# codeslake/RefVSR

Measured on AMD Instinct MI355X. Metric: 4x SR frames/sec (270p->1080p, RefVSR_small_L1), higher is better.
Workload: dtype f16; 1 GPU; config_RefVSR_small_L1 4x SR, 270x480 -> 1080x1920, frame_num=5, steady-state sliding window, n=1 (BASELINE configs[1]); synthetic clip seed 0, seeded random weights 1234; frames_per_rank=20, parallelism=frame-shard x1 (reset-aligned, no collective), window_cache=True, frame_ids=True, pipelined_calls=True, frames_per_call=4, headline_mode=frame groups, pipe_layout=pfm, full=False

## Files before the change

include/refvsr_hip.h:

```cpp
#ifndef REFVSR_HIP_H
#define REFVSR_HIP_H

#include <stddef.h>
#include <stdint.h>

#ifdef __cplusplus
extern "C" {
#endif

#define REFVSR_ABI_VERSION 15

int refvsr_abi_version(void);
int refvsr_max_maps(void);
const char* refvsr_last_error(void);
int refvsr_init(void);

int refvsr_num_cus(void);
int refvsr_stream_create_cu_range(int first_cu, int n_cus, void** stream);
int refvsr_stream_set_cu_budget(void* stream, int n_cus);
int refvsr_stream_destroy(void* stream);

enum { REFVSR_OUT_NHWC16 = 0, REFVSR_OUT_NHWC16_SHUFFLE2 = 1, REFVSR_OUT_PLANAR32 = 2 };

typedef struct RefvsrConv {
// ... 108 lines not shown
int refvsr_conf_alpha_f16w(const float* conf_a, const float* conf_b, int h, int w, int up, const float* w0, const float* b0,
                           float slope0, const void* blob, int cout, float slope1, void* alpha, float* conf_max, void* stream);
int refvsr_conf_alpha_batch_f16w(const float* const* conf_a, const float* const* conf_b, int batch, int h, int w, int up, const float* w0,
                                 const float* b0, float slope0, const void* blob, int cout, float slope1, void* const* alpha,
                                 float* const* conf_max, void* stream);
int refvsr_set_probe(void* buf, int iter);

int refvsr_conv_direct_f32(const float* src, int cin, int h, int w,
                           const float* wgt, const float* bias, int cout, int ksize, int stride, int pad,
                           float act_slope, void* out, int out_nhwc16, int out_c, void* stream);
int refvsr_conv1x1_f32(const float* src, int cin, int h, int w, const float* wgt, const float* bias, float act_slope,
                       float* out, void* stream);

int refvsr_pack_nhwc16(const float* src, int c, int h, int w, void* dst, int cs, void* stream);
int refvsr_pack_nhwc32(const float* src, int c, int h, int w, float* dst, int cs, void* stream);
int refvsr_unpack_nhwc16(const void* src, int h, int w, int cs, int c, float* dst, void* stream);

enum { REFVSR_RS_BICUBIC = 0, REFVSR_RS_BILINEAR = 1, REFVSR_RS_BILINEAR_AC = 2, REFVSR_RS_NEAREST = 3 };
int refvsr_resize(const float* src, int c, int h, int w, void* dst, int oh, int ow, int mode,
                  float src_scale_y, float src_scale_x, const float* mean, const float* std,
                  const float* chan_mul, int clamp01, int out_nhwc16, int out_c, void* stream);
int refvsr_avgpool2(const float* src, int c, int h, int w, float* dst, void* stream);
int refvsr_maxpool2(const float* src, int c, int h, int w, float* dst, void* stream);
int refvsr_buffers_equal(const void* const* a, const void* const* b, int n_pairs, size_t n_bytes,
                         int32_t* flags, void* stream);
int refvsr_bytes_equal(const void* const* a, const void* const* b, int n_pairs, size_t n_bytes,
                       int32_t* flags, void* stream);
int refvsr_max2(const float* a, const float* b, float* out, size_t n, void* stream);

#define REFVSR_INGEST_MAX_FRAMES 16
enum { REFVSR_INGEST_PLANAR = 0, REFVSR_INGEST_HWC = 1 };
int refvsr_ingest_u8(const void* const* src, float* const* dst, int nframes, int h, int w, int layout, void* stream);
int refvsr_ingest_table(float* out);
int refvsr_ingest_max_frames(void);

#define REFVSR_SCORE_MAX_FRAMES 16
size_t refvsr_score_workspace_bytes(int nframes, int h, int w);
int refvsr_score_max_frames(void);
int refvsr_score_frames(const void* const* out, int out_fmt, const void* const* gt, int gt_fmt, int gt_layout, int nframes, int h, int w,
                        int win, void* workspace, size_t workspace_bytes, double* scores, void* stream);

#define REFVSR_SCORE_MAX_RECTS 8
size_t refvsr_score_regions_workspace_bytes(int nframes, int h, int w, int nrects);
int refvsr_score_max_rects(void);
int refvsr_score_regions(const void* const* out, int out_fmt, const void* const* gt, int gt_fmt, int gt_layout, int nframes, int h, int w,
                         const int* rects, int nrects, void* workspace, size_t workspace_bytes, double* sums, void* stream);

int refvsr_warp_nhwc16(const void* x, int hin, int win, int cs, const float* flow, int hf, int wf,
                       void* out, void* stream);
int refvsr_warp_nhwc16_up2(const void* x, int hin, int win, int cs, const float* flow_lr, int hl, int wl,
                           void* out, void* stream);
int refvsr_warp_planar(const float* x, int c, int hin, int win, const float* flow, int hf, int wf,
                       float* out, void* stream);
int refvsr_warp_nhwc16_batch(const void* const* x, int batch, int hin, int win, int cs, const float* const* flow, int hf, int wf,
                             void* const* out, void* stream);
int refvsr_warp_nhwc16_up2_batch(const void* const* x, int batch, int hin, int win, int cs, const float* const* flow_lr, int hl, int wl,
                                 void* const* out, void* stream);
int refvsr_warp_planar_batch(const float* const* x, int batch, int c, int hin, int win, const float* const* flow, int hf, int wf,
                             float* const* out, void* stream);
int refvsr_spynet_level_input(const float* ref, const float* supp, const float* flow_prev, int h, int w,
                              void* out8, float* flow_up, void* stream);
int refvsr_spynet_level_input_batch(const float* const* ref, const float* const* supp, int batch, const float* flow_prev,
                                    int h, int w, void* out8, float* flow_up, void* stream);

#define REFVSR_MATCH_KP 152
#define REFVSR_MATCH_ROWCHUNK 256
#define REFVSR_MATCH_COLBLOCK 512
int refvsr_match_patches(const float* feat, int h, int w, void* rows, float* inv_norm, void* rows_lo, void* stream);
int refvsr_match_top2(const void* ref_rows, int n_ref, const void* lr_rows, int n_lr, int row_splits,
                      int32_t* cand_idx, float* cand_val, void* stream);
int refvsr_match_refine(const float* lr_feat, int h, int w, const float* ref_feat, int hr, int wr,
                        const float* inv_lr, const float* inv_ref, const int32_t* cand_idx, const float* cand_val,
                        int ncand, float margin, int32_t* flagged, float* conf, int32_t* idx, void* stream);
int refvsr_match_exact(const float* lr_feat, int h, int w, const float* ref_feat, int hr, int wr, const void* lr_rows,
                       const void* lr_rows_lo, const void* ref_rows, const void* ref_rows_lo, const float* inv_lr,
                       const float* inv_ref, const int32_t* flagged, void* keys, float* conf, int32_t* idx, void* stream);
int refvsr_match_naive(const float* lr_feat, int h, int w, const float* ref_feat, int hr, int wr,
                       float* conf, int32_t* idx, void* stream);

int refvsr_block_gather_nhwc16(const void* value, int hv, int wv, int cs, const int32_t* idx, int gh, int gw,
                               int s, void* out, void* stream);
int refvsr_block_gather_rgb(const float* value, int hv, int wv, const int32_t* idx, int gh, int gw, int s,
                            void* out8, float* out_planar, void* stream);
int refvsr_aligned_sample(const void* x, int h, int w, int ks, int cs, const float* affine, void* out,
                          void* stream);

int refvsr_dcn_sample(const void* x, int h, int w, int c, const float* offset_mask, int deform_groups, void* cols,
                      void* stream);
int refvsr_tsa_weight(const void* const* aligned, const void* const* emb, const void* emb_ref, int t, int c, int npix,
                      void* out, void* stream);
int refvsr_pool3s2_nhwc16(const void* x, int h, int w, int c, void* out, int out_c, int c_off, int is_max, void* stream);
// ... 8 lines not shown
```

refvsr_amd/csrc/match.hip:

```cpp
#include <stdlib.h>

#include "match_common.h"

#define LO_SCALE 2048.0f
#define LO_UNSCALE (1.0f / 2048.0f)

__global__ __launch_bounds__(128) void match_patches_kernel(const float* __restrict__ feat, int h, int w,
                                                            f16* __restrict__ rows, float* __restrict__ inv_norm,
                                                            f16* __restrict__ rows_lo) {
    __shared__ float s_inv[128];
    const int tid = threadIdx.x, p0 = blockIdx.x * 128, n = h * w;
    const size_t plane = (size_t)h * w;
    {
        const int p = min(p0 + tid, n - 1);
        const int y = p / w, x = p - y * w;
        int yy[3], xx[3];
#pragma unroll
        for (int k = 0; k < 3; ++k) { yy[k] = rv_reflect(y + k - 1, h) * w; xx[k] = rv_reflect(x + k - 1, w); }
        float ss = 0.0f;
        for (int c = 0; c < 16; ++c) {
            const float* f = feat + c * plane;
#pragma unroll
            for (int ky = 0; ky < 3; ++ky)
#pragma unroll
// ... 11 lines not shown
        const int y = p / w, x = p - y * w;
        const float inv = s_inv[pl];
        f16x8 o, lo;
#pragma unroll
        for (int k = 0; k < 8; ++k) {
            const int e = g * 8 + k;
            float v = 0.0f;
            if (e < 144) {
                const int c = e / 9, t = e - c * 9;
                const int ky = t / 3, kx = t - ky * 3;
                v = feat[c * plane + (size_t)rv_reflect(y + ky - 1, h) * w + rv_reflect(x + kx - 1, w)];
            }
            float vn = v * inv;
            asm volatile("" : "+v"(vn));
            o[k] = (f16)vn;
            lo[k] = (f16)((vn - (float)o[k]) * LO_SCALE);
        }
        const size_t off = (size_t)p0 * KP + (size_t)i * 8;
        *reinterpret_cast<f16x8*>(rows + off) = o;
        if (rows_lo) *reinterpret_cast<f16x8*>(rows_lo + off) = lo;
    }
}

extern "C" int refvsr_match_patches(const float* feat, int h, int w, void* rows, float* inv_norm, void* rows_lo,
                                    void* stream) {
    RV_CHECK(feat && rows && inv_norm && h >= 2 && w >= 2, "match_patches: bad args");
    hipLaunchKernelGGL(match_patches_kernel, dim3(rv_cdiv(h * w, 128)), dim3(128), 0, (hipStream_t)stream,
                       feat, h, w, (f16*)rows, inv_norm, (f16*)rows_lo);
    RV_LAUNCH_CHECK();
    return 0;
}

template <int UNROLL = 1>
__device__ __forceinline__ float patch_dot(const float* __restrict__ lf, int h, int w, const int* ly, const int* lx,
                                           const float* __restrict__ rf, int hr, int wr, int ry, int rx) {
    int yy[3], xx[3];
#pragma unroll
    for (int k = 0; k < 3; ++k) { yy[k] = rv_reflect(ry + k - 1, hr); xx[k] = rv_reflect(rx + k - 1, wr); }
    const size_t lp = (size_t)h * w, rp = (size_t)hr * wr;
    float d = 0.0f;
#pragma unroll 1
    for (int c0 = 0; c0 < 16; c0 += UNROLL) {
        float a[UNROLL][9], b[UNROLL][9];
#pragma unroll
        for (int u = 0; u < UNROLL; ++u)
#pragma unroll
            for (int t = 0; t < 9; ++t) {
                a[u][t] = lf[(c0 + u) * lp + (size_t)ly[t / 3] * w + lx[t % 3]];
                b[u][t] = rf[(c0 + u) * rp + (size_t)yy[t / 3] * wr + xx[t % 3]];
            }
#pragma unroll
// ... 265 lines not shown
```

refvsr_amd/engine.py:

```python
import collections
import itertools
import os

import torch

from . import ops
from .config import resolve_weight_precision
from .knobs import env_flag
from .packing import pack_conv
from .weights import VGG_MEAN, VGG_STD, round16

_uid = itertools.count()


def _timed_event(stream):
    e = torch.cuda.Event(enable_timing=True)
    e.record(stream)
    return e


def _flow_pairs(fr, restart):
    t = len(fr)
    ctr = t // 2
    need = [(fr[i], fr[i + 1]) for i in range(ctr, t - 1)] + [(fr[ctr + 1], fr[ctr])]
# ... 153 lines not shown
        self.nb = config.num_blocks
        self.ks = config.matching_ksize
        self.hd = bool(config.flag_HD_in)
        self.vgg7 = self.hd or config.scale != 4
        self.cache = bool(getattr(config, 'cache_windows', True))
        self.match_row_splits = 1
        self.match_margin = float(getattr(config, 'match_exact_margin', ops.MATCH_EXACT_MARGIN))
        self.chain_calls = bool(getattr(config, 'chain_calls', not env_flag('REFVSR_NO_CHAIN_CALLS')))
        self.fuse_resblocks = (bool(getattr(config, 'fuse_resblocks', True)) and ops.resblock_fits(self.C)
                               and not env_flag('REFVSR_NO_FUSE'))
        self.rb24 = not env_flag('REFVSR_NO_RB24')
        self.rb48 = (bool(getattr(config, 'fuse_resblocks', True)) and not env_flag('REFVSR_NO_FUSE')
                     and not env_flag('REFVSR_NO_RB48'))
        self.rb48_max_pixels = int(os.environ.get('REFVSR_RB48_MAX_PIXELS', str(540 * 960)))
        self.rb48_multimap = not env_flag('REFVSR_NO_RB48_MULTIMAP')
        self.spynet_mt1_pixels = int(os.environ.get('REFVSR_SPYNET_MT1_PIXELS', str(72 * 120)))
        self.bw_head_blocks = min(self.nb, max(-1, int(getattr(config, 'bw_head_blocks', None) if getattr(config, 'bw_head_blocks', None) is not None
                                                         else os.environ.get('REFVSR_BW_HEAD_BLOCKS', '12'))))
        self.warp_up2 = not env_flag('REFVSR_NO_WARP_UP2')
        self.fuse_head = not env_flag('REFVSR_NO_FUSE_HEAD')
        self.fuse_tail = self.fuse_head and (env_flag('REFVSR_FUSE_TAIL') or bool(getattr(config, 'fuse_tail', False)))
        self.fuse_conf = not env_flag('REFVSR_NO_FUSE_CONF')
        self.map1x1 = not env_flag('REFVSR_NO_MAP1X1')
        self.spynet_batch = not env_flag('REFVSR_NO_SPYNET_BATCH')
        self.overlap = bool(getattr(config, 'overlap_streams', True)) and not env_flag('REFVSR_NO_OVERLAP')
        self._side = None
        self.pipelined = bool(getattr(config, 'pipelined', False))
        self._zero_maps = {}
        self.result_dtype = str(getattr(config, 'result_dtype', None) or 'float32').replace('torch.', '')
        ops.result_format(self.result_dtype)
        self._pipe = None
        self._layout_default = None
        self.pipe_depth = max(1, int(getattr(config, 'pipe_depth', None) or os.environ.get('REFVSR_PIPE_DEPTH') or 3))
        self._inflight = collections.deque()
        self.stream_events = None
        self.kernel_events = None
        self.chain_events = None
        self.reset_state()

    def reset_state(self):
        self.fw_feat = None
        self.fw_flow = None
        self.fw_feat_up = None
        self.fw_conf = None
        self.frame_itr_num = 0
        self.max_frame_itr_num = self.cfg.reset_branch
# ... 256 lines not shown

    def res_list(self, x, name, n):
        pairs = [(self.cw('%s.RBs.%d.conv1' % (name, i)), self.cw('%s.RBs.%d.conv2' % (name, i))) for i in range(n)]
        y = self._block_chain(x, pairs, 0.2)
        return ops.conv(self.cw(name + '.conv_tail'), y, res=x)

    def resblocks(self, lr8, feat, name, stop=None, resume=None):
        pairs = [(self.cw('%s.main.2.%d.conv1' % (name, i)), self.cw('%s.main.2.%d.conv2' % (name, i)))
                 for i in range(self.nb)]
        if resume is not None:
            n, x = resume
            return self._block_chain(x, pairs[n:], 0.0) if n < self.nb else x
        x = ops.conv(self.cw(name + '.main.0'), lr8, feat, act=0.1)
        if stop is not None:
            return self._block_chain(x, pairs[:stop], 0.0) if stop > 0 else x
        return self._block_chain(x, pairs, 0.0)

    def pyramid(self, fr):
        if fr.pyr is None:
            h, w = fr.lr.shape[1:]
            w_up = w if w % 32 == 0 else 32 * (w // 32 + 1)
            h_up = h if h % 32 == 0 else 32 * (h // 32 + 1)
            lv = [ops.resize(fr.lr, (h_up, w_up), ops.RS_BILINEAR, mean=VGG_MEAN, std=VGG_STD)]
            for _ in range(5):
                lv.append(ops.avgpool2(lv[-1]))
            fr.pyr = lv[::-1]
        return fr.pyr

    def flow(self, fr_ref, fr_supp, share=None):
        key = (fr_ref.uid, fr_supp.uid)
        hit = self.flow_cache.get(key)
        if hit is not None:
            out, ev = hit
            if ev is not None:
                torch.cuda.current_stream().wait_event(ev)
                out.record_stream(torch.cuda.current_stream())
            return out
        for f in (fr_ref, fr_supp):
            if f.ready is not None:
                torch.cuda.current_stream().wait_event(f.ready)
        pr, ps = self.pyramid(fr_ref), self.pyramid(fr_supp)
        h, w = fr_ref.lr.shape[1:]
        flow = None
        for lvl in range(6):
            x, fup = ops.spynet_level_input(pr[lvl], ps[lvl], flow)
            p = 'FlowNet.basic_module.%d.basic_module.' % lvl
            small = x.shape[0] * x.shape[1] <= self.spynet_mt1_pixels
            for j in range(4):
# ... 36 lines not shown
        flow = None
        for lvl in range(6):
            x, fup = ops.spynet_level_input_batch([p_[lvl] for p_ in pr], [p_[lvl] for p_ in ps], flow)
            p = 'FlowNet.basic_module.%d.basic_module.' % lvl
            small = x.shape[1] * x.shape[2] <= self.spynet_mt1_pixels
            for j in range(4):
                cw = self.W.conv.get(p + '%d.conv/mt1' % j) if small else None
                x = ops.conv(cw if cw is not None else self.cw(p + '%d.conv' % j), x, act=0.0, batch=B)
            flow = ops.conv(self.cw(p + '4.conv'), x, planar_out=True, res_planar=fup, batch=B)
        h_up, w_up = flow.shape[2:]
        cm = [float(w) / float(w_up), float(h) / float(h_up)]
        outs = [ops.resize(flow[b0:b0 + 2].reshape(-1, h_up, w_up), (h, w), ops.RS_BILINEAR, chan_mul=cm * min(2, B - b0))
                for b0 in range(0, B, 2)]
        out = outs[0].view(-1, 2, h, w) if len(outs) == 1 else torch.cat([o_.view(-1, 2, h, w) for o_ in outs], 0)
        ev = None
        if share:
            ev = torch.cuda.Event()
            ev.record()
            for st in share:
                out.record_stream(st)
        for i, (a, b) in enumerate(todo):
            self.flow_cache[(a.uid, b.uid)] = (out[i], ev)

    def feature_match(self, fr):
        R = self.W.raw
        h, w = fr.lr.shape[1:]

        fe = 'feature_match.feature_extract.'

        def extract(x):
            x = ops.pack_nhwc32(x, 4)
            x = ops.conv(self.cw(fe + '0'), x, act=0.0)
            if not self.vgg7:
                x = ops.conv(self.cw(fe + '2'), x, act=0.0)
                if self.map1x1:
                    return ops.conv1x1_f32(x, *R[fe + 'map64.0'], act=0.2)
                return ops.conv(self.cw(fe + 'map64.0'), x, act=0.2, planar_out=True)
            x = ops.conv(self.cw(fe + '2'), x, act=0.0, planar_out=True)
            x = ops.pack_nhwc32(ops.maxpool2(x))
            x = ops.conv(self.cw(fe + '5'), x, act=0.0)
            if self.map1x1:
                return ops.conv1x1_f32(x, *R[fe + 'map128.0'], act=0.2)
            return ops.conv(self.cw(fe + 'map128.0'), x, act=0.2, planar_out=True)
        lr_n = ops.conv_direct(fr.lr, *R['feature_match.sub_mean'])
        ref_n = ops.conv_direct(fr.ref, *R['feature_match.sub_mean'])
        if self.hd:
            f = 1.0 / (self.cfg.scale // 2)
            oh, ow = int(h * f), int(w * f)
            lr_n = ops.resize(lr_n, (oh, ow), ops.RS_NEAREST, (1.0 / f, 1.0 / f))
            ref_n = ops.resize(ref_n, (oh, ow), ops.RS_NEAREST, (1.0 / f, 1.0 / f))
        lr_f = extract(lr_n)
        ref_f = extract(ops.avgpool2(ref_n))
        lr_rows, inv_lr, lr_lo = ops.match_patches(lr_f, ops.hip.MATCH_COLBLOCK, want_lo=True)
        ref_rows, inv_ref, ref_lo = ops.match_patches(ref_f, ops.hip.MATCH_ROWCHUNK, want_lo=True)
        n_lr = lr_f.shape[1] * lr_f.shape[2]
        n_ref = ref_f.shape[1] * ref_f.shape[2]
        if self.kernel_events is not None:
            e0, e1 = torch.cuda.Event(enable_timing=True), torch.cuda.Event(enable_timing=True)
            e0.record()
        cand, cand_val = ops.match_top2(ref_rows, n_ref, lr_rows, n_lr, self.match_row_splits)
        if self.kernel_events is not None:
            e1.record()
            self.kernel_events.append((e0, e1))
        conf, idx, _ = ops.match_refine(lr_f, ref_f, inv_lr, inv_ref, cand, cand_val, self.match_margin, (lr_rows, lr_lo),
                                        (ref_rows, ref_lo))
        conf = conf.view(1, lr_f.shape[1], lr_f.shape[2])
        grid = (lr_f.shape[1], lr_f.shape[2])
        if grid[0] != h:
            conf = ops.bicubic_scale(conf, float(h) / grid[0], clamp01=True)
        return conf, idx, grid

    def aligned_conv(self, feats, query, rgb8, prefix, ks):
        def enc(z8):
            e = ops.conv(self.cw(prefix + '.conv1.0'), z8, act=0.2)
            t = ops.conv(self.cw(prefix + '.conv1.2.conv1'), e, act=0.2)
            return ops.conv(self.cw(prefix + '.conv1.2.conv2'), t, res=e, post=0.2)
        q = enc(ops.bicubic_scale(query, 2, clamp01=False, nhwc16_out=True))
        r = enc(rgb8)
        a = ops.conv(self.cw(prefix + '.p_conv.0'), r, q, stride=ks, act=0.2)
        t = ops.conv(self.cw(prefix + '.p_conv.2.conv1'), a, act=0.2)
        a = ops.conv(self.cw(prefix + '.p_conv.2.conv2'), t, res=a, post=0.2)
        affine = ops.conv(self.cw(prefix + '.p_conv.4'), a, planar_out=True, add_const=1.0, clamp=(-3.0, 3.0))
        return ops.aligned_sample(feats, affine, ks)

    def _ref_encoders(self, fr):
        ref8 = ops.pack_nhwc16(fr.ref, 8)
        x = ops.conv(self.cw('ref_encoder1.0.0'), ref8, act=0.2)
        x = ops.conv(self.cw('ref_encoder1.1.0'), x, act=0.2)
        ref_feat = self.res_list(x, 'res1', 4)
        x = ops.conv(self.cw('ref_encoder2.0.0'), ref_feat, stride=2, act=0.2)
        x = ops.conv(self.cw('ref_encoder2.1.0'), x, act=0.2)
        return ref_feat, self.res_list(x, 'res2', 4)

    def prepare_frame(self, fr):
        if fr.conf is not None:
            return
        if self.ctx_strict:
            raise RuntimeError('a window needs a per-frame context that was neither prepared ahead nor imported (strict mode)')
        h, w = fr.lr.shape[1:]
        fr.lr8 = ops.pack_nhwc16(fr.lr, 8)
        fr.conf, fr.idx, (gh, gw) = self.feature_match(fr)
        ref_feat, ref_feat_down = self._ref_encoders(fr)
        s1, s2 = self.ks // 2, self.ks
        feats1 = ops.block_gather_nhwc16(ref_feat_down, fr.idx, gh, gw, s1)
        if s1 > 1:
            rgb1 = ops.block_gather_rgb(fr.ref, fr.idx, gh, gw, s1)
            lr_down = ops.bicubic_scale(fr.lr, 0.5, clamp01=True)
            fr.aligned = self.aligned_conv(feats1, lr_down, rgb1, 'aa1.align', s1)
        else:
            fr.aligned = feats1
        feats2 = ops.block_gather_nhwc16(ref_feat, fr.idx, gh, gw, s2)
        rgb2 = ops.block_gather_rgb(fr.ref, fr.idx, gh, gw, s2)
        fr.aligned_up = self.aligned_conv(feats2, fr.lr, rgb2, 'aa2.align', s2)

    def rap(self, fr, conf_prop, feat, feat_up):
        R = self.W.raw
        fused = self.fuse_conf and ops.conf_alpha_ok(self.cw('conf_fusion.1.0')) and ops.conf_alpha_ok(self.cw('conf_fusion2.1.0'))
        if fused:
            alpha, conf_next = ops.conf_alpha(conf_prop, fr.conf, 1, *R['conf_fusion.0.0'], self.cw('conf_fusion.1.0'), want_max=True)
        else:
            pair = torch.cat([conf_prop, fr.conf], 0)
            a = ops.conv_direct(pair, *R['conf_fusion.0.0'], act=0.2, nhwc16_out=True)
            alpha = ops.conv(self.cw('conf_fusion.1.0'), a, act=0.2)
        t = ops.conv(self.cw('feat_fusion.0.0'), feat, fr.aligned, act=0.2)
        feat = ops.conv(self.cw('feat_fusion.1.0'), t, act=0.2, mul=alpha, res=feat)
# ... 820 lines not shown
```

refvsr_amd/hip.py:

```python
import ctypes as C
import os

_HERE = os.path.dirname(os.path.abspath(__file__))
LIB_PATH = os.path.join(_HERE, 'librefvsr_hip.so')

OUT_NHWC16, OUT_NHWC16_SHUFFLE2, OUT_PLANAR32 = 0, 1, 2
RS_BICUBIC, RS_BILINEAR, RS_BILINEAR_AC, RS_NEAREST = 0, 1, 2, 3
RESULT_F32, RESULT_F16, RESULT_U8 = 0, 1, 2
INGEST_PLANAR, INGEST_HWC = 0, 1
MATCH_KP, MATCH_ROWCHUNK, MATCH_COLBLOCK = 152, 256, 512
ABI_VERSION = 15
MAX_MAPS = 4
INGEST_MAX_FRAMES = 16
SCORE_MAX_FRAMES = 16
SCORE_MAX_RECTS = 8
RESBLOCK24_BLOB_BYTES = 43264
RESBLOCK24_F16W_BLOB_BYTES = 28928
RESBLOCK48_BLOB_BYTES = 172544


class RefvsrConv(C.Structure):
    _fields_ = [
        ('src0', C.c_void_p), ('c0', C.c_int),
        ('src1', C.c_void_p), ('c1', C.c_int),
# ... 96 lines not shown
    'refvsr_up2_bilinear_nhwc16': [_P, _I, _I, _I, _F, _P, _P],
    'refvsr_tsa_blend': [_P, _P, _P, _Z, _P, _P],
    'refvsr_resblock24_f16w_blob_bytes': [],
    'refvsr_conv24_f16w_blob_bytes': [_I, _I],
    'refvsr_conv32_f16w_blob_bytes': [_I, _I],
    'refvsr_conv_shuffle2_f16w_blob_bytes': [_I],
    'refvsr_resblock24_chain_f16w': [_P, _I, _I, _I, _P, _Z, _F, _P, _P, _P, _P],
    'refvsr_resblock24_chain_batch_f16w': [_P, _I, _I, _I, _I, _P, _Z, _F, _P, _P, _P, _P],
    'refvsr_conv24_f16w': [_P, _I, _P, _I, _I, _I, _P, _F, _P, _P, _F, _P, _P],
    'refvsr_conv24_batch_f16w': [_P, _I, _P, _I, _I, _I, _I, _P, _F, _P, _P, _F, _P, _P],
    'refvsr_conv32_f16w': [_P, _I, _P, _I, _I, _I, _P, _F, _P, _P, _F, _P, _P],
    'refvsr_conv_shuffle2_f16w': [_P, _I, _I, _I, _P, _F, _P, _P],
    'refvsr_conv_shuffle2_batch_f16w': [_P, _I, _I, _I, _I, _P, _F, _P, _P],
    'refvsr_conf_alpha_f16w': [_P, _P, _I, _I, _I, _P, _P, _F, _P, _I, _F, _P, _P, _P],
    'refvsr_conf_alpha_batch_f16w': [_P, _P, _I, _I, _I, _I, _P, _P, _F, _P, _I, _F, _P, _P, _P],
    'refvsr_ingest_u8': [_P, _P, _I, _I, _I, _I, _P],
    'refvsr_ingest_table': [_P],
    'refvsr_ingest_max_frames': [],
    'refvsr_bytes_equal': [_P, _P, _I, _Z, _P, _P],
    'refvsr_score_frames': [_P, _I, _P, _I, _I, _I, _I, _I, _I, _P, _Z, _P, _P],
    'refvsr_score_max_frames': [],
    'refvsr_score_regions': [_P, _I, _P, _I, _I, _I, _I, _I, _P, _I, _P, _Z, _P, _P],
    'refvsr_score_max_rects': [],
}
_SPECIAL = {'refvsr_abi_version': (C.c_int, []), 'refvsr_last_error': (C.c_char_p, []),
            'refvsr_score_workspace_bytes': (C.c_size_t, [_I, _I, _I]),
            'refvsr_score_regions_workspace_bytes': (C.c_size_t, [_I, _I, _I, _I])}
EXPORTS = tuple(sorted(list(SIGNATURES) + list(_SPECIAL)))

_lib = None


def lib():
    global _lib
    if _lib is None:
        if not os.path.exists(LIB_PATH):
            raise RuntimeError(
                'refvsr_amd: %s not found -- the HIP extension is required (no CPU fallback). '
                'Build it with `make -C refvsr_amd/csrc` or `python -c "import __graft_entry__ as g; g.build()"`.'
                % LIB_PATH)
        h = C.CDLL(LIB_PATH)
        for name, args in SIGNATURES.items():
            fn = getattr(h, name)
            fn.argtypes = args
            fn.restype = C.c_int
        for name, (res, args) in _SPECIAL.items():
# ... 25 lines not shown
```

refvsr_amd/ops.py:

```python
import ctypes as C
import math
import os

import torch

from . import hip
from .knobs import env_flag
from .hip import (OUT_NHWC16, OUT_NHWC16_SHUFFLE2, OUT_PLANAR32, RS_BICUBIC, RS_BILINEAR,
                  RS_BILINEAR_AC, RS_NEAREST)


_STREAM = None


def _stream():
    if _STREAM is not None:
        return _STREAM
    return C.c_void_p(torch.cuda.current_stream().cuda_stream)


class on_stream(object):

    def __init__(self, stream):
        self.stream = stream
# ... 495 lines not shown
    return out


def bicubic_scale(x, factor, clamp01=True, nhwc16_out=False):
    c, h, w = x.shape
    oh, ow = int(math.floor(h * factor)), int(math.floor(w * factor))
    s = 1.0 / factor
    return resize(x, (oh, ow), RS_BICUBIC, (s, s), clamp01=clamp01, nhwc16_out=nhwc16_out)


def flow_up2(flow):
    c, h, w = flow.shape
    return resize(flow, (2 * h, 2 * w), RS_BILINEAR_AC, (0.0, 0.0), chan_mul=[2.0] * c)


def avgpool2(x):
    _planar(x)
    c, h, w = x.shape
    out = torch.empty((c, h // 2, w // 2), dtype=torch.float32, device=x.device)
    hip.check(hip.lib().refvsr_avgpool2(_ptr(x), c, h, w, _ptr(out), _stream()), 'avgpool2')
    return out


def maxpool2(x):
    _planar(x)
    c, h, w = x.shape
    out = torch.empty((c, h // 2, w // 2), dtype=torch.float32, device=x.device)
    hip.check(hip.lib().refvsr_maxpool2(_ptr(x), c, h, w, _ptr(out), _stream()), 'maxpool2')
    return out


def max2(a, b):
    assert a.shape == b.shape and a.dtype == torch.float32 and a.is_contiguous() and b.is_contiguous()
    out = torch.empty_like(a)
    hip.check(hip.lib().refvsr_max2(_ptr(a), _ptr(b), _ptr(out), a.numel(), _stream()), 'max2')
    return out


def buffers_equal(pairs):
    if not pairs:
        return []
    nbytes = pairs[0][0].numel() * 4
    flags = torch.ones(len(pairs), dtype=torch.int32, device=pairs[0][0].device)
    for s0 in range(0, len(pairs), 32):
        chunk = pairs[s0:s0 + 32]
        for a, b in chunk:
# ... 186 lines not shown
    hip.check(hip.lib().refvsr_spynet_level_input(_ptr(ref), _ptr(supp), _ptr(flow_prev), h, w, _ptr(out8), _ptr(fup),
                                                  _stream()), 'spynet_level_input')
    return out8, fup


def spynet_level_input_batch(refs, supps, flow_prev):
    B = len(refs)
    assert 1 <= B <= 8 and len(supps) == B
    for t_ in list(refs) + list(supps):
        _planar(t_, 3)
    h, w = refs[0].shape[1:]
    if flow_prev is not None:
        assert flow_prev.is_cuda and flow_prev.dtype == torch.float32 and flow_prev.is_contiguous() and \
            tuple(flow_prev.shape) == (B, 2, h // 2, w // 2)
    out8 = torch.empty((B, h, w, 8), dtype=torch.float16, device=refs[0].device)
    fup = torch.empty((B, 2, h, w), dtype=torch.float32, device=refs[0].device)
    pr = (C.c_void_p * B)(*[t_.data_ptr() for t_ in refs])
    ps = (C.c_void_p * B)(*[t_.data_ptr() for t_ in supps])
    hip.check(hip.lib().refvsr_spynet_level_input_batch(pr, ps, B, _ptr(flow_prev), h, w, _ptr(out8), _ptr(fup), _stream()),
              'spynet_level_input_batch')
    return out8, fup


def match_patches(feat, row_pad, want_lo=False):
    _planar(feat, 16)
    h, w = feat.shape[1:]
    n = h * w
    rows = torch.empty((_round_up(n, row_pad), hip.MATCH_KP), dtype=torch.float16, device=feat.device)
    inv = torch.empty((n,), dtype=torch.float32, device=feat.device)
    lo = torch.empty_like(rows) if want_lo else None
    if rows.shape[0] > n:
        rows[n:].zero_()
        if lo is not None:
            lo[n:].zero_()
    hip.check(hip.lib().refvsr_match_patches(_ptr(feat), h, w, _ptr(rows), _ptr(inv), _ptr(lo), _stream()), 'match_patches')
    return (rows, inv, lo) if want_lo else (rows, inv)


def match_top2(ref_rows, n_ref, lr_rows, n_lr, row_splits=1):
    assert ref_rows.shape[0] % hip.MATCH_ROWCHUNK == 0 and lr_rows.shape[0] % hip.MATCH_COLBLOCK == 0
    assert ref_rows.shape[0] >= n_ref and lr_rows.shape[0] >= n_lr
    ci = torch.empty((n_lr, 2 * row_splits), dtype=torch.int32, device=ref_rows.device)
    cv = torch.empty((n_lr, 2 * row_splits), dtype=torch.float32, device=ref_rows.device)
    hip.check(hip.lib().refvsr_match_top2(_ptr(ref_rows), n_ref, _ptr(lr_rows), n_lr, row_splits, _ptr(ci), _ptr(cv),
                                          _stream()), 'match_top2')
    return ci, cv


MATCH_EXACT_MARGIN = 2.5e-4


def match_refine(lr_feat, ref_feat, inv_lr, inv_ref, cand, cand_val=None, margin=None, lr_split=None, ref_split=None):
    _planar(lr_feat, 16)
    _planar(ref_feat, 16)
    h, w = lr_feat.shape[1:]
    hr, wr = ref_feat.shape[1:]
    assert cand.dtype == torch.int32 and cand.shape[0] == h * w and cand.is_contiguous()
    conf = torch.empty((h * w,), dtype=torch.float32, device=lr_feat.device)
    idx = torch.empty((h * w,), dtype=torch.int32, device=lr_feat.device)
    if margin is None:
        hip.check(hip.lib().refvsr_match_refine(_ptr(lr_feat), h, w, _ptr(ref_feat), hr, wr, _ptr(inv_lr), _ptr(inv_ref),
                                                _ptr(cand), None, cand.shape[1], 0.0, None, _ptr(conf), _ptr(idx), _stream()),
                  'match_refine')
        return conf, idx
    assert cand_val is not None and ref_split is not None and lr_split is not None
    assert cand_val.shape == cand.shape and cand_val.is_contiguous()
    (lr_rows, lr_lo), (ref_rows, ref_lo) = lr_split, ref_split
    for r, n_, pad in ((lr_rows, h * w, 1), (lr_lo, h * w, 1), (ref_rows, hr * wr, hip.MATCH_ROWCHUNK), (ref_lo, hr * wr, hip.MATCH_ROWCHUNK)):
        assert r.dtype == torch.float16 and r.is_contiguous() and r.shape[1] == hip.MATCH_KP
        assert r.shape[0] >= n_ and r.shape[0] % pad == 0
    n = h * w
    fl_words = (n + 2) // 2 * 2
    scratch = torch.zeros(fl_words + 2 * n, dtype=torch.int32, device=lr_feat.device)
    flagged, keys = scratch[:n + 1], scratch[fl_words:]
    hip.check(hip.lib().refvsr_match_refine(_ptr(lr_feat), h, w, _ptr(ref_feat), hr, wr, _ptr(inv_lr), _ptr(inv_ref),
                                            _ptr(cand), _ptr(cand_val), cand.shape[1], float(margin), _ptr(flagged), _ptr(conf),
                                            _ptr(idx), _stream()), 'match_refine')
    hip.check(hip.lib().refvsr_match_exact(_ptr(lr_feat), h, w, _ptr(ref_feat), hr, wr, _ptr(lr_rows), _ptr(lr_lo), _ptr(ref_rows), _ptr(ref_lo),
                                           _ptr(inv_lr), _ptr(inv_ref), _ptr(flagged), _ptr(keys), _ptr(conf), _ptr(idx),
                                           _stream()), 'match_exact')
    return conf, idx, flagged


def match_naive(lr_feat, ref_feat):
    _planar(lr_feat, 16)
    _planar(ref_feat, 16)
    h, w = lr_feat.shape[1:]
    hr, wr = ref_feat.shape[1:]
    conf = torch.empty((h * w,), dtype=torch.float32, device=lr_feat.device)
    idx = torch.empty((h * w,), dtype=torch.int32, device=lr_feat.device)
    hip.check(hip.lib().refvsr_match_naive(_ptr(lr_feat), h, w, _ptr(ref_feat), hr, wr, _ptr(conf), _ptr(idx),
                                           _stream()), 'match_naive')
    return conf, idx


def block_gather_nhwc16(value, idx, gh, gw, s):
    _nhwc(value)
    hv, wv, cs = value.shape
    assert idx.dtype == torch.int32 and idx.numel() == gh * gw and idx.is_contiguous()
    out = torch.empty((gh * s, gw * s, cs), dtype=torch.float16, device=value.device)
# ... 223 lines not shown
```

Measured before the change: 228.6 frames/s.

## Fuse frame prep, pyramid pooling, LDS patch extraction, sparse low rows

```diff
diff --git a/include/refvsr_hip.h b/include/refvsr_hip.h
--- a/include/refvsr_hip.h
+++ b/include/refvsr_hip.h
@@ -154,6 +154,9 @@
                   const float* chan_mul, int clamp01, int out_nhwc16, int out_c, void* stream);
 int refvsr_avgpool2(const float* src, int c, int h, int w, float* dst, void* stream);
 int refvsr_maxpool2(const float* src, int c, int h, int w, float* dst, void* stream);
+int refvsr_avgpool_pyramid(const float* src, int c, int h, int w, float* const* dst, void* stream);
+int refvsr_frame_prep(const float* lr, int h, int w, const float* ref, int hr, int wr, const float* wgt, const float* bias,
+                      void* lr8, void* ref8, float* lr_n, float* ref_n, void* stream);
 int refvsr_buffers_equal(const void* const* a, const void* const* b, int n_pairs, size_t n_bytes,
                          int32_t* flags, void* stream);
 int refvsr_bytes_equal(const void* const* a, const void* const* b, int n_pairs, size_t n_bytes,
@@ -199,6 +202,9 @@
 #define REFVSR_MATCH_ROWCHUNK 256
 #define REFVSR_MATCH_COLBLOCK 512
 int refvsr_match_patches(const float* feat, int h, int w, void* rows, float* inv_norm, void* rows_lo, void* stream);
+int refvsr_set_match_patches_kernel(int mode);
+int refvsr_match_lo_rows(const float* feat, int h, int w, const float* inv_norm, const int32_t* flagged, void* rows_lo,
+                         void* stream);
 int refvsr_match_top2(const void* ref_rows, int n_ref, const void* lr_rows, int n_lr, int row_splits,
                       int32_t* cand_idx, float* cand_val, void* stream);
 int refvsr_match_refine(const float* lr_feat, int h, int w, const float* ref_feat, int hr, int wr,
diff --git a/refvsr_amd/csrc/match.hip b/refvsr_amd/csrc/match.hip
--- a/refvsr_amd/csrc/match.hip
+++ b/refvsr_amd/csrc/match.hip
@@ -57,11 +57,135 @@
     }
 }
 
+#define MP_S 256
+#define MP_LD (MP_S + 2)
+__global__ __launch_bounds__(256) void match_patches_lds_kernel(const float* __restrict__ feat, int h, int w,
+                                                                f16* __restrict__ rows, float* __restrict__ inv_norm,
+                                                                f16* __restrict__ rows_lo) {
+    __shared__ float s_f[48 * MP_LD];
+    __shared__ float s_inv[MP_S];
+    __shared__ int s_edge[MP_S];
+    const int tid = threadIdx.x, p0 = blockIdx.x * MP_S, n = h * w;
+    const size_t plane = (size_t)h * w;
+    for (int j = tid; j < MP_LD; j += 256) {
+        const int q = min(max(p0 - 1 + j, 0), n - 1);
+        const int y = q / w, x = q - y * w;
+        int ro[3];
+#pragma unroll
+        for (int k = 0; k < 3; ++k) ro[k] = rv_reflect(y + k - 1, h) * w + x;
+#pragma unroll 4
+        for (int c = 0; c < 16; ++c) {
+            const float* f = feat + c * plane;
+#pragma unroll
+            for (int ky = 0; ky < 3; ++ky) s_f[(c * 3 + ky) * MP_LD + j] = f[ro[ky]];
+        }
+    }
+    __syncthreads();
+    {
+        const int p = min(p0 + tid, n - 1);
+        const int x = p % w;
+        const int edge = (x == 0 ? 1 : 0) | (x == w - 1 ? 2 : 0);
+        const float* sp = s_f + (p - p0) + 1;
+        const int d0 = (edge & 1) ? 1 : -1, d2 = (edge & 2) ? -1 : 1;
+        float ss = 0.0f;
+#pragma unroll 4
+        for (int r = 0; r < 48; ++r) {
+            const float v0 = sp[r * MP_LD + d0], v1 = sp[r * MP_LD], v2 = sp[r * MP_LD + d2];
+            ss = fmaf(v0, v0, ss);
+            ss = fmaf(v1, v1, ss);
+            ss = fmaf(v2, v2, ss);
+        }
+        const float inv = 1.0f / fmaxf(sqrtf(ss), 1e-12f);
+        s_inv[tid] = inv;
+        s_edge[tid] = edge;
+        if (p0 + tid < n) inv_norm[p0 + tid] = inv;
+    }
+    __syncthreads();
+    const int n_slots = min(MP_S, n - p0) * 19;
+    for (int i = tid; i < n_slots; i += 256) {
+        const int pl = i / 19, g = i - pl * 19;
+        const float inv = s_inv[pl];
+        const int edge = s_edge[pl];
+        int r = (g * 8) / 3, kx = g * 8 - r * 3;
+        const float* sp = s_f + r * MP_LD + pl + 1;
+        f16x8 o, lo;
+#pragma unroll
+        for (int k = 0; k < 8; ++k) {
+            float v = 0.0f;
+            if (g < 18) {
+                const int d = kx == 0 ? ((edge & 1) ? 1 : -1) : kx == 1 ? 0 : ((edge & 2) ? -1 : 1);
+                v = sp[d];
+            }
+            if (++kx == 3) { kx = 0; sp += MP_LD; }
+            float vn = v * inv;
+            asm volatile("" : "+v"(vn));
+            o[k] = (f16)vn;
+            lo[k] = (f16)((vn - (float)o[k]) * LO_SCALE);
+        }
+        const size_t off = (size_t)p0 * KP + (size_t)i * 8;
+        *reinterpret_cast<f16x8*>(rows + off) = o;
+        if (rows_lo) *reinterpret_cast<f16x8*>(rows_lo + off) = lo;
+    }
+}
+
+static int g_match_patches_kernel = 1;
+extern "C" int refvsr_set_match_patches_kernel(int mode) {
+    if (mode < 0 || mode > 1) return 1;
+    g_match_patches_kernel = mode;
+    return 0;
+}
+
 extern "C" int refvsr_match_patches(const float* feat, int h, int w, void* rows, float* inv_norm, void* rows_lo,
                                     void* stream) {
     RV_CHECK(feat && rows && inv_norm && h >= 2 && w >= 2, "match_patches: bad args");
-    hipLaunchKernelGGL(match_patches_kernel, dim3(rv_cdiv(h * w, 128)), dim3(128), 0, (hipStream_t)stream,
-                       feat, h, w, (f16*)rows, inv_norm, (f16*)rows_lo);
+    RV_CHECK((long long)h * w <= (1ll << 26), "match_patches: map too large");
+    if (g_match_patches_kernel == 1)
+        hipLaunchKernelGGL(match_patches_lds_kernel, dim3(rv_cdiv(h * w, MP_S)), dim3(256), 0, (hipStream_t)stream,
+                           feat, h, w, (f16*)rows, inv_norm, (f16*)rows_lo);
+    else
+        hipLaunchKernelGGL(match_patches_kernel, dim3(rv_cdiv(h * w, 128)), dim3(128), 0, (hipStream_t)stream,
+                           feat, h, w, (f16*)rows, inv_norm, (f16*)rows_lo);
+    RV_LAUNCH_CHECK();
+    return 0;
+}
+
+__global__ __launch_bounds__(256) void match_lo_rows_kernel(const float* __restrict__ feat, int h, int w,
+                                                            const float* __restrict__ inv_norm,
+                                                            const int32_t* __restrict__ flagged, f16* __restrict__ rows_lo) {
+    const int total = flagged[0] * 19;
+    const size_t plane = (size_t)h * w;
+    for (int i = blockIdx.x * 256 + threadIdx.x; i < total; i += gridDim.x * 256) {
+        const int f = i / 19, g = i - f * 19;
+        const int p = flagged[1 + f];
+        const int y = p / w, x = p - y * w;
+        const float inv = inv_norm[p];
+        f16x8 lo;
+#pragma unroll
+        for (int k = 0; k < 8; ++k) {
+            const int e = g * 8 + k;
+            float v = 0.0f;
+            if (e < 144) {
+                const int c = e / 9, t = e - c * 9;
+                const int ky = t / 3, kx = t - ky * 3;
+                v = feat[c * plane + (size_t)rv_reflect(y + ky - 1, h) * w + rv_reflect(x + kx - 1, w)];
+            }
+            float vn = v * inv;
+            asm volatile("" : "+v"(vn));
+            const f16 hi = (f16)vn;
+            lo[k] = (f16)((vn - (float)hi) * LO_SCALE);
+        }
+        *reinterpret_cast<f16x8*>(rows_lo + (size_t)p * KP + g * 8) = lo;
+    }
+}
+
+extern "C" int refvsr_match_lo_rows(const float* feat, int h, int w, const float* inv_norm, const int32_t* flagged,
+                                    void* rows_lo, void* stream) {
+    RV_CHECK(feat && inv_norm && flagged && rows_lo && h >= 2 && w >= 2, "match_lo_rows: bad args");
+    RV_CHECK((long long)h * w <= (1ll << 26), "match_lo_rows: map too large");
+    const int slots = rv_cdiv(h * w * 19, 256);
+    const int grid = slots < 1024 ? slots : 1024;
+    hipLaunchKernelGGL(match_lo_rows_kernel, dim3(grid), dim3(256), 0, (hipStream_t)stream, feat, h, w, inv_norm, flagged,
+                       (f16*)rows_lo);
     RV_LAUNCH_CHECK();
     return 0;
 }
diff --git a/refvsr_amd/csrc/prep.hip b/refvsr_amd/csrc/prep.hip
--- /dev/null
+++ b/refvsr_amd/csrc/prep.hip
@@ -0,0 +1,148 @@
+#include "common.h"
+
+struct PyrArgs { const float* src; float* dst[5]; int h, w; };
+
+__device__ __forceinline__ float pool4(float a, float b, float cc, float d) {
+#pragma clang fp contract(off)
+    return 0.25f * (a + b + cc + d);
+}
+
+__global__ __launch_bounds__(256) void avgpool_pyramid_kernel(PyrArgs a) {
+    __shared__ float s1[16 * 16], s2[8 * 8], s3[4 * 4], s4[2 * 2];
+    const int tid = threadIdx.x;
+    const int tx = blockIdx.x, ty = blockIdx.y, ch = blockIdx.z;
+    const int h = a.h, w = a.w;
+    {
+        const int ox = tid & 15, oy = tid >> 4;
+        const float* s = a.src + ((size_t)ch * h + ty * 32 + 2 * oy) * w + tx * 32 + 2 * ox;
+        const float2 r0 = *reinterpret_cast<const float2*>(s), r1 = *reinterpret_cast<const float2*>(s + w);
+        const float v = pool4(r0.x, r0.y, r1.x, r1.y);
+        a.dst[0][((size_t)ch * (h >> 1) + ty * 16 + oy) * (w >> 1) + tx * 16 + ox] = v;
+        s1[tid] = v;
+    }
+    __syncthreads();
+    if (tid < 64) {
+        const int ox = tid & 7, oy = tid >> 3;
+        const float* s = s1 + (2 * oy) * 16 + 2 * ox;
+        const float v = pool4(s[0], s[1], s[16], s[17]);
+        a.dst[1][((size_t)ch * (h >> 2) + ty * 8 + oy) * (w >> 2) + tx * 8 + ox] = v;
+        s2[tid] = v;
+    }
+    __syncthreads();
+    if (tid < 16) {
+        const int ox = tid & 3, oy = tid >> 2;
+        const float* s = s2 + (2 * oy) * 8 + 2 * ox;
+        const float v = pool4(s[0], s[1], s[8], s[9]);
+        a.dst[2][((size_t)ch * (h >> 3) + ty * 4 + oy) * (w >> 3) + tx * 4 + ox] = v;
+        s3[tid] = v;
+    }
+    __syncthreads();
+    if (tid < 4) {
+        const int ox = tid & 1, oy = tid >> 1;
+        const float* s = s3 + (2 * oy) * 4 + 2 * ox;
+        const float v = pool4(s[0], s[1], s[4], s[5]);
+        a.dst[3][((size_t)ch * (h >> 4) + ty * 2 + oy) * (w >> 4) + tx * 2 + ox] = v;
+        s4[tid] = v;
+    }
+    __syncthreads();
+    if (tid == 0) a.dst[4][((size_t)ch * (h >> 5) + ty) * (w >> 5) + tx] = pool4(s4[0], s4[1], s4[2], s4[3]);
+}
+
+extern "C" int refvsr_avgpool_pyramid(const float* src, int c, int h, int w, float* const* dst, void* stream) {
+    RV_CHECK(src && dst && c > 0 && c <= 65535 && h > 0 && w > 0, "avgpool_pyramid: bad args");
+    RV_CHECK(h % 32 == 0 && w % 32 == 0 && h / 32 <= 65535, "avgpool_pyramid: the map must be a whole number of 32 x 32 tiles (got %d x %d)", h, w);
+    RV_CHECK(((uintptr_t)src & 7) == 0, "avgpool_pyramid: src must be 8-byte aligned");
+    PyrArgs a;
+    a.src = src; a.h = h; a.w = w;
+    for (int k = 0; k < 5; ++k) {
+        RV_CHECK(dst[k], "avgpool_pyramid: null level pointer (level %d)", k + 1);
+        a.dst[k] = dst[k];
+    }
+    hipLaunchKernelGGL(avgpool_pyramid_kernel, dim3(w / 32, h / 32, c), dim3(256), 0, (hipStream_t)stream, a);
+    RV_LAUNCH_CHECK();
+    return 0;
+}
+
+struct PrepArgs {
+    const float* lr; const float* ref; const float* wgt; const float* bias;
+    f16* lr8; f16* ref8; float* lr_n; float* ref_n;
+    int h, w, hr, wr;
+};
+
+__device__ __forceinline__ void mean_shift3(const float (&x)[3], const float (&wg)[9], const float (&b)[3], float (&o)[3]) {
+#pragma clang fp contract(off)
+#pragma unroll
+    for (int co = 0; co < 3; ++co) {
+        float acc = 0.0f;
+#pragma unroll
+        for (int ci = 0; ci < 3; ++ci) acc = fmaf(x[ci], wg[co * 3 + ci], acc);
+        o[co] = rv_lrelu(acc + b[co], 1.0f);
+    }
+}
+
+__device__ __forceinline__ f16x8 pack8(const float (&x)[3]) {
+    f16x8 v;
+#pragma unroll
+    for (int k = 0; k < 8; ++k) v[k] = (f16)0.f;
+#pragma unroll
+    for (int k = 0; k < 3; ++k) v[k] = (f16)x[k];
+    return v;
+}
+
+__global__ __launch_bounds__(256) void frame_prep_kernel(PrepArgs a) {
+    const int n_lr = a.h * a.w;
+    const int qw = (a.wr + 1) >> 1, qh = (a.hr + 1) >> 1;
+    const int i = blockIdx.x * 256 + threadIdx.x;
+    if (i >= n_lr + qw * qh) return;
+    float wg[9], b[3];
+#pragma unroll
+    for (int k = 0; k < 9; ++k) wg[k] = a.wgt[k];
+#pragma unroll
+    for (int k = 0; k < 3; ++k) b[k] = a.bias[k];
+    if (i < n_lr) {
+        float x[3], m[3];
+#pragma unroll
+        for (int ch = 0; ch < 3; ++ch) x[ch] = a.lr[(size_t)ch * n_lr + i];
+        mean_shift3(x, wg, b, m);
+        *reinterpret_cast<f16x8*>(a.lr8 + (size_t)i * 8) = pack8(x);
+        *reinterpret_cast<f32x4*>(a.lr_n + (size_t)i * 4) = (f32x4){m[0], m[1], m[2], 0.f};
+        return;
+    }
+    const int q = i - n_lr;
+    const int qy = q / qw, qx = q - qy * qw;
+    const size_t plane = (size_t)a.hr * a.wr;
+    float m[4][3];
+#pragma unroll
+    for (int t = 0; t < 4; ++t) {
+        const int y = 2 * qy + (t >> 1), x_ = 2 * qx + (t & 1);
+        if (y < a.hr && x_ < a.wr) {
+            const size_t pix = (size_t)y * a.wr + x_;
+            float x[3];
+#pragma unroll
+            for (int ch = 0; ch < 3; ++ch) x[ch] = a.ref[ch * plane + pix];
+            mean_shift3(x, wg, b, m[t]);
+            *reinterpret_cast<f16x8*>(a.ref8 + pix * 8) = pack8(x);
+        }
+    }
+    if (2 * qy + 1 < a.hr && 2 * qx + 1 < a.wr) {
+        float* o = a.ref_n + ((size_t)qy * (a.wr >> 1) + qx) * 4;
+        *reinterpret_cast<f32x4*>(o) = (f32x4){pool4(m[0][0], m[1][0], m[2][0], m[3][0]), pool4(m[0][1], m[1][1], m[2][1], m[3][1]),
+                                               pool4(m[0][2], m[1][2], m[2][2], m[3][2]), 0.f};
+    }
+}
+
+extern "C" int refvsr_frame_prep(const float* lr, int h, int w, const float* ref, int hr, int wr, const float* wgt, const float* bias,
+                                 void* lr8, void* ref8, float* lr_n, float* ref_n, void* stream) {
+    RV_CHECK(lr && ref && wgt && bias && lr8 && ref8 && lr_n && ref_n, "frame_prep: null pointer");
+    RV_CHECK(h > 0 && w > 0 && hr >= 2 && wr >= 2, "frame_prep: bad sizes");
+    RV_CHECK((long long)h * w + (long long)((hr + 1) / 2) * ((wr + 1) / 2) < (1ll << 30), "frame_prep: frames too large");
+    RV_CHECK((((uintptr_t)lr8 | (uintptr_t)ref8 | (uintptr_t)lr_n | (uintptr_t)ref_n) & 15) == 0, "frame_prep: outputs must be 16-byte aligned");
+    PrepArgs a;
+    a.lr = lr; a.ref = ref; a.wgt = wgt; a.bias = bias;
+    a.lr8 = (f16*)lr8; a.ref8 = (f16*)ref8; a.lr_n = lr_n; a.ref_n = ref_n;
+    a.h = h; a.w = w; a.hr = hr; a.wr = wr;
+    const int total = h * w + ((hr + 1) / 2) * ((wr + 1) / 2);
+    hipLaunchKernelGGL(frame_prep_kernel, dim3(rv_cdiv(total, 256)), dim3(256), 0, (hipStream_t)stream, a);
+    RV_LAUNCH_CHECK();
+    return 0;
+}
diff --git a/refvsr_amd/engine.py b/refvsr_amd/engine.py
--- a/refvsr_amd/engine.py
+++ b/refvsr_amd/engine.py
@@ -199,6 +199,8 @@
         self.fuse_tail = self.fuse_head and (env_flag('REFVSR_FUSE_TAIL') or bool(getattr(config, 'fuse_tail', False)))
         self.fuse_conf = not env_flag('REFVSR_NO_FUSE_CONF')
         self.map1x1 = not env_flag('REFVSR_NO_MAP1X1')
+        self.legacy_prep = env_flag('REFVSR_LEGACY_PREP')
+        self.last_flagged = None
         self.spynet_batch = not env_flag('REFVSR_NO_SPYNET_BATCH')
         self.overlap = bool(getattr(config, 'overlap_streams', True)) and not env_flag('REFVSR_NO_OVERLAP')
         self._side = None
@@ -501,8 +503,11 @@
             w_up = w if w % 32 == 0 else 32 * (w // 32 + 1)
             h_up = h if h % 32 == 0 else 32 * (h // 32 + 1)
             lv = [ops.resize(fr.lr, (h_up, w_up), ops.RS_BILINEAR, mean=VGG_MEAN, std=VGG_STD)]
-            for _ in range(5):
-                lv.append(ops.avgpool2(lv[-1]))
+            if self.legacy_prep:
+                for _ in range(5):
+                    lv.append(ops.avgpool2(lv[-1]))
+            else:
+                lv += ops.avgpool_pyramid(lv[0])
             fr.pyr = lv[::-1]
         return fr.pyr
 
@@ -585,14 +590,18 @@
         for i, (a, b) in enumerate(todo):
             self.flow_cache[(a.uid, b.uid)] = (out[i], ev)
 
-    def feature_match(self, fr):
+    def frame_prep(self, fr):
+        if self.hd or self.legacy_prep:
+            return None
+        return ops.frame_prep(fr.lr, fr.ref, *self.W.raw['feature_match.sub_mean'])
+
+    def feature_match(self, fr, prep=None):
         R = self.W.raw
         h, w = fr.lr.shape[1:]
 
         fe = 'feature_match.feature_extract.'
 
         def extract(x):
-            x = ops.pack_nhwc32(x, 4)
             x = ops.conv(self.cw(fe + '0'), x, act=0.0)
             if not self.vgg7:
                 x = ops.conv(self.cw(fe + '2'), x, act=0.0)
@@ -605,16 +614,26 @@
             if self.map1x1:
                 return ops.conv1x1_f32(x, *R[fe + 'map128.0'], act=0.2)
             return ops.conv(self.cw(fe + 'map128.0'), x, act=0.2, planar_out=True)
-        lr_n = ops.conv_direct(fr.lr, *R['feature_match.sub_mean'])
-        ref_n = ops.conv_direct(fr.ref, *R['feature_match.sub_mean'])
-        if self.hd:
-            f = 1.0 / (self.cfg.scale // 2)
-            oh, ow = int(h * f), int(w * f)
-            lr_n = ops.resize(lr_n, (oh, ow), ops.RS_NEAREST, (1.0 / f, 1.0 / f))
-            ref_n = ops.resize(ref_n, (oh, ow), ops.RS_NEAREST, (1.0 / f, 1.0 / f))
+        if prep is None:
+            prep = self.frame_prep(fr)
+        if prep is not None:
+            lr_n, ref_n = prep[2], prep[3]
+        else:
+            lr_n = ops.conv_direct(fr.lr, *R['feature_match.sub_mean'])
+            ref_n = ops.conv_direct(fr.ref, *R['feature_match.sub_mean'])
+            if self.hd:
+                f = 1.0 / (self.cfg.scale // 2)
+                oh, ow = int(h * f), int(w * f)
+                lr_n = ops.resize(lr_n, (oh, ow), ops.RS_NEAREST, (1.0 / f, 1.0 / f))
+                ref_n = ops.resize(ref_n, (oh, ow), ops.RS_NEAREST, (1.0 / f, 1.0 / f))
+            lr_n, ref_n = ops.pack_nhwc32(lr_n, 4), ops.pack_nhwc32(ops.avgpool2(ref_n), 4)
         lr_f = extract(lr_n)
-        ref_f = extract(ops.avgpool2(ref_n))
-        lr_rows, inv_lr, lr_lo = ops.match_patches(lr_f, ops.hip.MATCH_COLBLOCK, want_lo=True)
+        ref_f = extract(ref_n)
+        ops.set_match_patches_kernel(0 if self.legacy_prep else 1)
+        if self.legacy_prep:
+            lr_rows, inv_lr, lr_lo = ops.match_patches(lr_f, ops.hip.MATCH_COLBLOCK, want_lo=True)
+        else:
+            (lr_rows, inv_lr), lr_lo = ops.match_patches(lr_f, ops.hip.MATCH_COLBLOCK), None
         ref_rows, inv_ref, ref_lo = ops.match_patches(ref_f, ops.hip.MATCH_ROWCHUNK, want_lo=True)
         n_lr = lr_f.shape[1] * lr_f.shape[2]
         n_ref = ref_f.shape[1] * ref_f.shape[2]
@@ -625,8 +644,8 @@
         if self.kernel_events is not None:
             e1.record()
             self.kernel_events.append((e0, e1))
-        conf, idx, _ = ops.match_refine(lr_f, ref_f, inv_lr, inv_ref, cand, cand_val, self.match_margin, (lr_rows, lr_lo),
-                                        (ref_rows, ref_lo))
+        conf, idx, self.last_flagged = ops.match_refine(lr_f, ref_f, inv_lr, inv_ref, cand, cand_val, self.match_margin, (lr_rows, lr_lo),
+                                                        (ref_rows, ref_lo))
         conf = conf.view(1, lr_f.shape[1], lr_f.shape[2])
         grid = (lr_f.shape[1], lr_f.shape[2])
         if grid[0] != h:
@@ -646,8 +665,9 @@
         affine = ops.conv(self.cw(prefix + '.p_conv.4'), a, planar_out=True, add_const=1.0, clamp=(-3.0, 3.0))
         return ops.aligned_sample(feats, affine, ks)
 
-    def _ref_encoders(self, fr):
-        ref8 = ops.pack_nhwc16(fr.ref, 8)
+    def _ref_encoders(self, fr, ref8=None):
+        if ref8 is None:
+            ref8 = ops.pack_nhwc16(fr.ref, 8)
         x = ops.conv(self.cw('ref_encoder1.0.0'), ref8, act=0.2)
         x = ops.conv(self.cw('ref_encoder1.1.0'), x, act=0.2)
         ref_feat = self.res_list(x, 'res1', 4)
@@ -661,9 +681,10 @@
         if self.ctx_strict:
             raise RuntimeError('a window needs a per-frame context that was neither prepared ahead nor imported (strict mode)')
         h, w = fr.lr.shape[1:]
-        fr.lr8 = ops.pack_nhwc16(fr.lr, 8)
-        fr.conf, fr.idx, (gh, gw) = self.feature_match(fr)
-        ref_feat, ref_feat_down = self._ref_encoders(fr)
+        prep = self.frame_prep(fr)
+        fr.lr8 = prep[0] if prep is not None else ops.pack_nhwc16(fr.lr, 8)
+        fr.conf, fr.idx, (gh, gw) = self.feature_match(fr, prep)
+        ref_feat, ref_feat_down = self._ref_encoders(fr, prep[1] if prep is not None else None)
         s1, s2 = self.ks // 2, self.ks
         feats1 = ops.block_gather_nhwc16(ref_feat_down, fr.idx, gh, gw, s1)
         if s1 > 1:
diff --git a/refvsr_amd/hip.py b/refvsr_amd/hip.py
--- a/refvsr_amd/hip.py
+++ b/refvsr_amd/hip.py
@@ -142,6 +142,10 @@
     'refvsr_score_max_frames': [],
     'refvsr_score_regions': [_P, _I, _P, _I, _I, _I, _I, _I, _P, _I, _P, _Z, _P, _P],
     'refvsr_score_max_rects': [],
+    'refvsr_set_match_patches_kernel': [_I],
+    'refvsr_match_lo_rows': [_P, _I, _I, _P, _P, _P, _P],
+    'refvsr_avgpool_pyramid': [_P, _I, _I, _I, _P, _P],
+    'refvsr_frame_prep': [_P, _I, _I, _P, _I, _I, _P, _P, _P, _P, _P, _P, _P],
 }
 _SPECIAL = {'refvsr_abi_version': (C.c_int, []), 'refvsr_last_error': (C.c_char_p, []),
             'refvsr_score_workspace_bytes': (C.c_size_t, [_I, _I, _I]),
diff --git a/refvsr_amd/ops.py b/refvsr_amd/ops.py
--- a/refvsr_amd/ops.py
+++ b/refvsr_amd/ops.py
@@ -541,6 +541,37 @@
     return out
 
 
+def avgpool_pyramid(x):
+    _planar(x)
+    c, h, w = x.shape
+    assert h % 32 == 0 and w % 32 == 0
+    sizes = [c * (h >> k) * (w >> k) for k in range(1, 6)]
+    offs = [0]
+    for n in sizes:
+        offs.append(offs[-1] + (n + 63) // 64 * 64)
+    buf = torch.empty((offs[-1],), dtype=torch.float32, device=x.device)
+    lv = [buf[offs[k]:offs[k] + sizes[k]].view(c, h >> (k + 1), w >> (k + 1)) for k in range(5)]
+    dst = (C.c_void_p * 5)(*[t_.data_ptr() for t_ in lv])
+    hip.check(hip.lib().refvsr_avgpool_pyramid(_ptr(x), c, h, w, dst, _stream()), 'avgpool_pyramid')
+    return lv
+
+
+def frame_prep(lr, ref, w, b):
+    _planar(lr, 3)
+    _planar(ref, 3)
+    assert tuple(w.shape) == (3, 3, 1, 1) and w.is_cuda and w.dtype == torch.float32 and w.is_contiguous()
+    assert tuple(b.shape) == (3,) and b.is_cuda and b.dtype == torch.float32 and b.is_contiguous()
+    h, wd = lr.shape[1:]
+    hr, wr = ref.shape[1:]
+    lr8 = torch.empty((h, wd, 8), dtype=torch.float16, device=lr.device)
+    ref8 = torch.empty((hr, wr, 8), dtype=torch.float16, device=lr.device)
+    lr_n = torch.empty((h, wd, 4), dtype=torch.float32, device=lr.device)
+    ref_n = torch.empty((hr // 2, wr // 2, 4), dtype=torch.float32, device=lr.device)
+    hip.check(hip.lib().refvsr_frame_prep(_ptr(lr), h, wd, _ptr(ref), hr, wr, _ptr(w), _ptr(b), _ptr(lr8), _ptr(ref8), _ptr(lr_n),
+                                          _ptr(ref_n), _stream()), 'frame_prep')
+    return lr8, ref8, lr_n, ref_n
+
+
 def maxpool2(x):
     _planar(x)
     c, h, w = x.shape
@@ -773,6 +804,10 @@
     return out8, fup
 
 
+def set_match_patches_kernel(mode):
+    hip.check(hip.lib().refvsr_set_match_patches_kernel(int(mode)), 'set_match_patches_kernel')
+
+
 def match_patches(feat, row_pad, want_lo=False):
     _planar(feat, 16)
     h, w = feat.shape[1:]
@@ -817,6 +852,9 @@
     assert cand_val is not None and ref_split is not None and lr_split is not None
     assert cand_val.shape == cand.shape and cand_val.is_contiguous()
     (lr_rows, lr_lo), (ref_rows, ref_lo) = lr_split, ref_split
+    sparse_lo = lr_lo is None
+    if sparse_lo:
+        lr_lo = torch.empty_like(lr_rows)
     for r, n_, pad in ((lr_rows, h * w, 1), (lr_lo, h * w, 1), (ref_rows, hr * wr, hip.MATCH_ROWCHUNK), (ref_lo, hr * wr, hip.MATCH_ROWCHUNK)):
         assert r.dtype == torch.float16 and r.is_contiguous() and r.shape[1] == hip.MATCH_KP
         assert r.shape[0] >= n_ and r.shape[0] % pad == 0
@@ -827,6 +865,8 @@
     hip.check(hip.lib().refvsr_match_refine(_ptr(lr_feat), h, w, _ptr(ref_feat), hr, wr, _ptr(inv_lr), _ptr(inv_ref),
                                             _ptr(cand), _ptr(cand_val), cand.shape[1], float(margin), _ptr(flagged), _ptr(conf),
                                             _ptr(idx), _stream()), 'match_refine')
+    if sparse_lo:
+        hip.check(hip.lib().refvsr_match_lo_rows(_ptr(lr_feat), h, w, _ptr(inv_lr), _ptr(flagged), _ptr(lr_lo), _stream()), 'match_lo_rows')
     hip.check(hip.lib().refvsr_match_exact(_ptr(lr_feat), h, w, _ptr(ref_feat), hr, wr, _ptr(lr_rows), _ptr(lr_lo), _ptr(ref_rows), _ptr(ref_lo),
                                            _ptr(inv_lr), _ptr(inv_ref), _ptr(flagged), _ptr(keys), _ptr(conf), _ptr(idx),
                                            _stream()), 'match_exact')
```

Result: faster. 232.7 frames/s (median of 6 runs) (+1.8%).
